# hungkq-1724/EraXviF5TTS

Measured on AMD Instinct MI355X. Metric: mel-frames/s, higher is better.
Workload: dtype bf16; 1 GPU; C2 F5TTS_Base random-init, CFM.sample euler NFE=32 CFG=2 sway=-1, 32 utterances x seq_len 1024 (N_ref=341), one GPU, hipGraph=on; global_batch=32, per_gpu_batch=32, seq_len=1024, nfe=32, parallelism=utterance-sharded dp1, residual_stream=fp16 storage, fp32 arithmetic

## Files before the change

eraxvif5tts_amd/_lib.py:

```python
from __future__ import annotations

import ctypes as C
import os

import torch

_HERE = os.path.dirname(os.path.abspath(__file__))
LIB_PATH = os.environ.get("F5HIP_LIB") or os.path.join(_HERE, "lib", "libf5hip.so")

F5_PREC_BF16, F5_PREC_FP32, F5_PREC_FP16 = 0, 1, 2
PRECISIONS = {"bf16": F5_PREC_BF16, "fp32": F5_PREC_FP32, "fp16": F5_PREC_FP16}
F5_ODE_EULER, F5_ODE_MIDPOINT, F5_ODE_RK4, F5_ODE_HEUN2, F5_ODE_HEUN3 = 0, 1, 2, 3, 4
ODE_METHODS = {"euler": F5_ODE_EULER, "midpoint": F5_ODE_MIDPOINT, "rk4": F5_ODE_RK4, "heun2": F5_ODE_HEUN2, "heun3": F5_ODE_HEUN3}
F5_ROPE_ADJACENT, F5_ROPE_HALF_SPLIT = 0, 1
F5_BACKBONE_DIT, F5_BACKBONE_UNETT, F5_BACKBONE_MMDIT = 0, 1, 2
F5_SKIP = {"concat": 0, "add": 1, "none": 2}
SITES = ("qkv", "attention", "attn_out", "ff1", "ff2", "ln1", "ln2", "conv31", "input_proj")
F5_MEL_VOCOS, F5_MEL_BIGVGAN = 0, 1
ACT = {"none": 0, "gelu_tanh": 1, "gelu_erf": 2, "mish": 3}


class F5HipError(RuntimeError):
    pass

# ... 63 lines not shown
    "f5_sample_masked": (_I, [_P, _I, _I, _P, _P, _I, _P, _P, _P, _P, _I, _F, _I, _P, _P, _P, _I, _P]),
    "f5_sample_finish": (_I, [_P, _P]),
    "f5_text_embed": (_I, [_P, _I, _I, _P, _I, _I, _P, _P]),
    "f5_dit_forward": (_I, [_P, _I, _I, _P, _P, _P, _P, _I, _P, _P, _P]),
    "f5_sample_ragged": (_I, [_P, _I, _P, _P, _P, _I, _P, _P, _P, _I, C.c_float, _I, _P, _P]),
    "f5_sample_ragged_ex": (_I, [_P, _I, _P, _P, _P, _I, _P, _P, _P, _P, _I, C.c_float, _P, _I, _P, _P]),
    "f5_mmdit_forward": (_I, [_P, _I, _I, _I, _P, _P, _P, _P, _I, _P, _P, _P]),
    "f5_cfm_noise": (_I, [_I, _I, _I, _P, _P, _P, _P, _P, _P, _P]),
    "f5_cfm_loss_workspace": (C.c_int64, [_I, _I, _I]),
    "f5_cfm_loss": (_I, [_I, _I, _I, _P, _P, _P, _P, _P, _P, _P, _P, _P]),
    "f5_distill_loss_workspace": (C.c_int64, [_I, _I, _I]),
    "f5_distill_loss": (_I, [_I, _I, _I, _P, _P, _P, _P, _P, _P, _P, _P, _P, _P]),
    "f5_plan_set_blocks": (_I, [_P, _P, _I]),
    "f5_plan_get_blocks": (_I, [_P, _P, _I]),
    "f5_align_similarity":(_I, [_I, _I, _I, _I, _I, _I, _P, _P, _P, _P, _P, _P, _P, _P]),
    "f5_align_workspace": (C.c_int64, [_I, _I, _I]),
    "f5_align_viterbi": (_I, [_I, _I, _I, _P, _P, _P, _P, _P]),
    "f5_align_window": (_I, [_I, _I, _I, _P, _P, _P, _P, _P]),
    "f5_duration_loss": (_I, [_I, _I, _P, _P, _P, _P, _P, _P, _P, _P]),
    "f5_plan_timing_begin": (_I, [_P, _I]),
    "f5_plan_timing_end": (_I, [_P, C.POINTER(C.c_float), C.POINTER(C.c_int), _P]),
    "f5_plan_timing_site": (_I, [_P, _I, C.POINTER(C.c_float), C.POINTER(C.c_int)]),
    "f5_plan_set_tap": (_I, [_P, C.c_char_p, _P]),
    "f5_plan_set_option": (_I, [_P, C.c_char_p, _I]),
    "f5_plan_set_attn_dropout": (_I, [_P, _F, C.c_uint64]),
    "f5_plan_get_option": (_I, [_P, C.c_char_p, C.POINTER(C.c_int)]),
    "f5_duration_predict": (_I, [C.POINTER(DurationWeights), _I, _I, _P, _I, _P, _P, _P, _P]),
    "f5_duration_predict_g": (_I, [C.POINTER(DurationWeights), _I, _I, _P, _I, _P, _P, _I, _P, _P, _P]),
    "f5_op_linear": (_I, [_I, _I, _I, _I, _I, _P, _P, _P, _I, _P, _P]),
    "f5_op_linear_fused": (_I, [_I, _I, _I, _I, _I, _P, _P, _P, _I, _P, _P, _P, _I, _I, _P, _P]),
    "f5_op_ln_fold": (_I, [_I, _I, _I, _I, _I, _P, _P, _P, _P, _P, _P, _P, _P, _P, _P, _I, _P, _I, _I, _P, _P, _P]),
    "f5_op_linear_fused_p": (_I, [_I, _I, _I, _I, _I, _I, _P, _P, _P, _I, _P, _P, _P, _I, _I, _P, _P]),
    "f5_op_ln_fold_p": (_I, [_I, _I, _I, _I, _I, _I, _P, _P, _P, _P, _P, _P, _P, _P, _P, _P, _I, _P, _I, _I, _P, _P, _P]),
    "f5_op_layernorm_modulate": (_I, [_I, _I, _P, _P, _P, _P, _P]),
    "f5_op_attention": (_I, [_I, _I, _I, _I, _I, _P, _P, _P, _P]),
    "f5_op_attention_dropout": (_I, [_I, _I, _I, _I, _I, _P, _P, _F, C.c_uint64, C.c_uint32, C.c_uint32, _P, _P]),
    "f5_op_attention_prescaled": (_I, [_I, _I, _I, _I, _P, _P, _P, _P]),
    "f5_op_fold_weights": (_I, [_I, _I, _I, _I, _I, _P, _P, _P, _P, _P, _P, _P, _P, _P, _P]),
    "f5_op_attention_ragged": (_I, [_I, _I, _I, _I, C.POINTER(C.c_int), C.POINTER(C.c_int), _I, _I, _I, _I, _P, _P, _P]),
    "f5_op_conv_pos_embed": (_I, [_I, _I, _I, _I, _P, _P, _P, _P, _P, _P, _P]),
    "f5_op_conv31": (_I, [_I, _I, _I, _I, _I, _P, _P, _P, _I, _P, _P]),
    "f5_op_tile_gemm": (_I, [C.POINTER(TileGemm), _P]),
    "f5_op_layernorm_res": (_I, [_I, _I, _I, _I, _I, _I, _I, _I, _P, _P, _P, _I, _P, _P, _I, _I, _I, _I, _I, _P, _P, _P, _P]),
    "f5_op_f32_to_f16": (_I, [C.c_int64, _P, _P, _P, _P]),
    "f5_op_qknorm_rope": (_I, [_I, _I, _I, _I, _I, _P, _P, _P, _P, _P, _P]),
    "f5_op_dwconv7_ln": (_I, [_I, _I, _I, _I, _P, _P, _P, _P, _P, _P, _P]),
    "f5_op_grn": (_I, [_I, _I, _I, _I, _P, _P, _P, _P, _P]),
    "f5_op_rmsnorm": (_I, [_I, _I, _I, _P, _P, _P, _P]),
    "f5_bench_gemm_site": (_I, [_I, _I, _I, _I, _I, _I, _I, _I, C.POINTER(C.c_float), _P]),
    "f5_bench_attention": (_I, [_I, _I, _I, _I, _I, C.POINTER(C.c_float), _P]),
    "f5_bench_mfma_rate": (_I, [_I, C.POINTER(C.c_float), _P]),
    "f5_tuning_set": (_I, [C.c_char_p, _I]),
    "f5_tuning_get": (_I, [C.c_char_p, C.POINTER(C.c_int)]),
    "f5_tuning_key": (C.c_char_p, [_I]),
    "f5_debug_gemm_clock": (_I, [_P]),
    "f5_debug_last_gemm": (_I, [C.POINTER(C.c_int)] * 5),
    "f5_debug_eval_modes": (_I, [_P, _I, _I, _I, C.POINTER(C.c_int32)]),
    "f5_vocoder_create": (_I, [C.POINTER(VocosConfig), C.POINTER(_P)]),
    "f5_vocoder_set_tensor": (_I, [_P, C.c_char_p, _P, C.POINTER(C.c_int64), _I]),
    "f5_vocoder_has_tensor": (_I, [_P, C.c_char_p, C.POINTER(C.c_int64)]),
    "f5_vocoder_finalize": (_I, [_P]),
    "f5_vocoder_destroy": (_I, [_P]),
    "f5_vocoder_decode": (_I, [_P, _I, _I, _P, _P, _P]),
    "f5_vocoder_istft_head": (_I, [_P, _I, _I, _P, _P, _P]),
    "f5_vocoder_decode_ragged": (_I, [_P, _I, C.POINTER(C.c_int32), C.POINTER(C.c_int32), _P, _I, _P, C.POINTER(C.c_int64), _P]),
    "f5_wave_finish": (_I, [_I, _P, C.POINTER(C.c_int32), C.POINTER(C.c_float), C.POINTER(C.c_uint8), _P, C.c_float, _I, _I, _P, _P, _P, _P, _P,
# ... 124 lines not shown
```

eraxvif5tts_amd/csrc/gemm_w4.hip:

```cpp
#include "gemm_tile.h"
#include "lnf_stats_math.h"
#include "tuning.h"
#include <string.h>

typedef _Float16 f16x4_t __attribute__((ext_vector_type(4)));

namespace {
constexpr int OPB = 32768;
constexpr int EPI_LDS_BYTES = 16384;

template <int EPI, bool LNF, int MI, typename EL = bf16_t>
__global__ __launch_bounds__(256) __attribute__((amdgpu_waves_per_eu(1, 1))) void gemm_w4_kernel(GemmParams p, int tiles_n, int nblocks) {
    static_assert(EPI == EPI_STORE_T || EPI == EPI_ROPE_T || EPI == EPI_RESID, "block linears only");
    static_assert(!LNF || EPI != EPI_RESID, "LayerNorm fold: QKV (+ RoPE) and FF1 (+ GELU)");
    static_assert(MI == 8 || MI == 4, "token tiles per wave");
    constexpr int WROWS = MI * 16, BM = 2 * WROWS;
    constexpr int OPA = BM * 128;
    constexpr int WBASE = 2 * OPA, EPI_LDS = 2 * OPA + 2 * OPB;
    constexpr int NP = MI + 8, NR = MI + 8, NMF = 16 * MI;
    constexpr int LNF_AREA = MI == 4 ? 11264 : 2048;
    constexpr int EPI_BYTES = 4 * LNF_AREA > EPI_LDS_BYTES ? 4 * LNF_AREA : EPI_LDS_BYTES;
    constexpr bool WL = MI == 8 && EPI != EPI_RESID;
    __shared__ __attribute__((aligned(1024))) char smem[EPI_LDS + EPI_BYTES];
    const int tid = threadIdx.x, lane = tid & 63;
    const int wave = __builtin_amdgcn_readfirstlane(tid >> 6);
    const int wm = wave >> 1, wn = wave & 1;
    const int fr = lane & 15, fq = lane >> 4;

    auto tile_mn = [&](int bid, int& tm0, int& tn0) {
        const int q = nblocks >> 3, r = nblocks & 7, xcd = bid & 7;
        int swz = (xcd < r ? xcd * (q + 1) : r * (q + 1) + (xcd - r) * q) + (bid >> 3);
        if (p.tile_reverse) swz = nblocks - 1 - swz;
        const int gm = p.tile_group > 0 ? p.tile_group : 1;
        const int tiles_m_all = nblocks / tiles_n;
        const int grp = swz / (gm * tiles_n);
        const int gsz = min(gm, tiles_m_all - grp * gm);
        const int rin = swz - grp * gm * tiles_n;
        const int tile_n = rin / gsz, tile_m = grp * gm + (rin - tile_n * gsz);
        tm0 = tile_m * BM;
        tn0 = tile_n * 256;
    };
    [[maybe_unused]] unsigned pfv[4] = {0u, 0u, 0u, 0u};
    if constexpr (MI == 4) {
        if (p.pf_n[0] | p.pf_n[1]) {
#pragma unroll
            for (int r = 0; r < 2; ++r) {
                const size_t line = ((size_t)blockIdx.x * 2 + r) * 256u + tid;
                if (line * 128u < p.pf_n[0]) pfv[r] = *reinterpret_cast<const unsigned*>(static_cast<const char*>(p.pf_p[0]) + line * 128u);
                if (line * 128u < p.pf_n[1]) pfv[2 + r] = *reinterpret_cast<const unsigned*>(static_cast<const char*>(p.pf_p[1]) + line * 128u);
            }
        }
    }
    const int G = gridDim.x;
    const int my_tiles = (nblocks - (int)blockIdx.x + G - 1) / G;
    const int nk = p.K / 64;

    unsigned voffA[MI], voffW[8];
#pragma unroll
    for (int jj = 0; jj < 8; ++jj) {
        const int row = (wave * 8 + jj) * 8 + (lane >> 3);
        const int logical = (lane & 7) ^ ((row >> 1) & 7);
        const int wrow = WL ? (row & ~127) + 8 * (row & 15) + ((row & 127) >> 4) : row;
        voffW[jj] = (unsigned)(wrow * p.ldw * 2 + logical * 16);
    }
#pragma unroll
    for (int jj = 0; jj < MI; ++jj) {
        const int row = (wave * MI + jj) * 8 + (lane >> 3);
        const int logical = (lane & 7) ^ ((row >> 1) & 7);
        voffA[jj] = (unsigned)(row * p.lda * 2 + logical * 16);
    }
    const char* baseA;
    const char* baseW;
    int f_tile = blockIdx.x, f_k = 0;
    auto front_tile = [&]() {
        int sm, sn;
        tile_mn(f_tile, sm, sn);
        baseA = static_cast<const char*>(p.A) + (size_t)sm * p.lda * 2;
        baseW = static_cast<const char*>(p.W) + (size_t)sn * p.ldw * 2;
    };
    front_tile();
    const unsigned lds0 = (unsigned)(size_t)smem;
    const int wdstA = (int)lds0 + wave * MI * 1024, wdstW = (int)lds0 + WBASE + wave * 8192;
    auto dma16w = [&](int ldsdst, unsigned voff, const char* base) {
        asm volatile("s_mov_b32 m0, %0\n\ts_nop 0\n\tglobal_load_lds_dwordx4 %1, %2" ::"s"(ldsdst), "v"(voff), "s"(base) : "memory");
    };
    auto dma4w = [&](int ldsdst, unsigned voff, const void* base) {
        asm volatile("s_mov_b32 m0, %0\n\ts_nop 0\n\tglobal_load_lds_dword %1, %2" ::"s"(ldsdst), "v"(voff), "s"(base) : "memory");
    };
    auto front_advance = [&]() {
        baseA += 128;
        baseW += 128;
        if (++f_k == nk) {
            f_k = 0;
            f_tile += G;
            if (f_tile < nblocks) {
// ... 1 lines not shown
            } else {
                f_tile -= G;
                baseA -= (size_t)nk * 128;
                baseW -= (size_t)nk * 128;
            }
        }
    };
    const unsigned ra0 = lds0 + (unsigned)((wm * WROWS + fr) * 128 + ((fq ^ (fr >> 1)) * 16));
    const unsigned ra1 = ra0 ^ 64u;
    const unsigned rw0 = lds0 + WBASE + (unsigned)((wn * 128 + fr) * 128 + ((fq ^ (fr >> 1)) * 16));
    const unsigned rw1 = rw0 ^ 64u;

    f32x4 acc[8][MI];
    f32x4 fw[2][8], fa[2][MI];
#define W4_DSR(dst, addr, off) asm volatile("ds_read_b128 %0, %1 offset:%2" : "=v"(dst) : "v"(addr), "n"(off))
    auto rd = [&](auto sc, auto xc, auto ec) {
        constexpr int S = decltype(sc)::value, X = decltype(xc)::value, e = decltype(ec)::value;
        (void)fw; (void)fa; (void)ra0; (void)ra1; (void)rw0; (void)rw1;
        if constexpr (e < 8) {
            if constexpr (S == 0) W4_DSR(fw[0][e], rw0, X * OPB + e * 2048); else W4_DSR(fw[1][e], rw1, X * OPB + e * 2048);
        } else {
            if constexpr (S == 0) W4_DSR(fa[0][e - 8], ra0, X * OPA + (e - 8) * 2048); else W4_DSR(fa[1][e - 8], ra1, X * OPA + (e - 8) * 2048);
        }
    };
    auto body = [&](auto xc, auto waitc) {
        constexpr int X = decltype(xc)::value;
        constexpr bool WAITV = decltype(waitc)::value;
        constexpr int R1S = 1, B1P = MI == 8 ? 20 : 13, D0 = MI == 8 ? 22 : 14, DS = MI == 8 ? 6 : 4, B2P = MI == 8 ? 86 : 42, R0 = MI == 8 ? 88 : 44,
                      R0S = MI == 8 ? 2 : 1;
        static_for<NMF>([&](auto nc) {
            (void)acc; (void)fw; (void)fa; (void)voffA; (void)voffW; (void)baseA; (void)baseW;
            constexpr int n = decltype(nc)::value;
            constexpr int s = n / (8 * MI), i = (n % (8 * MI)) / MI, j = n % MI;
            if constexpr (WL) {
                if constexpr (LNF || Elem<EL>::F16)
                    asm volatile("v_mfma_f32_16x16x32_f16 %0, %1, %2, %0" : "+a"(acc[i][j]) : "v"(fa[s][j]), "v"(fw[s][i]));
                else
                    asm volatile("v_mfma_f32_16x16x32_bf16 %0, %1, %2, %0" : "+a"(acc[i][j]) : "v"(fa[s][j]), "v"(fw[s][i]));
            } else if constexpr (LNF || Elem<EL>::F16)
                asm volatile("v_mfma_f32_16x16x32_f16 %0, %1, %2, %0" : "+a"(acc[i][j]) : "v"(fw[s][i]), "v"(fa[s][j]));
            else
                asm volatile("v_mfma_f32_16x16x32_bf16 %0, %1, %2, %0" : "+a"(acc[i][j]) : "v"(fw[s][i]), "v"(fa[s][j]));
            if constexpr (n < NR * R1S && n % R1S == 0) rd(std::integral_constant<int, 1>{}, xc, std::integral_constant<int, n / R1S>{});
            if constexpr (n == B1P) asm volatile("s_waitcnt lgkmcnt(0)\n\ts_barrier" ::: "memory");
            if constexpr (n >= D0 && n < D0 + NP * DS && (n - D0) % DS == 0) {
                constexpr int pc = (n - D0) / DS;
                if constexpr (pc < MI)
                    dma16w(X * OPA + wdstA + pc * 1024, voffA[pc], baseA);
                else
                    dma16w(X * OPB + wdstW + (pc - MI) * 1024, voffW[pc - MI], baseW);
            }
            if constexpr (n == B2P) {
                constexpr int issued = (B2P - D0) / DS + 1 > NP ? NP : (B2P - D0) / DS + 1;
                if constexpr (WAITV)
                    asm volatile("s_waitcnt vmcnt(%0)\n\ts_barrier" ::"n"(issued) : "memory");
                else
                    asm volatile("s_barrier" ::: "memory");
            }
            if constexpr (n >= R0 && n < R0 + NR * R0S && (n - R0) % R0S == 0)
                rd(std::integral_constant<int, 0>{}, std::integral_constant<int, 1 - X>{}, std::integral_constant<int, (n - R0) / R0S>{});
            if constexpr (n == NMF - 1) asm volatile("s_waitcnt lgkmcnt(0)" ::: "memory");
        });
        front_advance();
    };

    using T = std::true_type;
    using F = std::false_type;
// ... 16 lines not shown
#pragma unroll
                    for (int c = 0; c < 16; ++c)
                        dma16w(ldst + 2048 + c * 512, ro, reinterpret_cast<const char*>(p.lnf_partial + (size_t)c * p.lnf_partial_ld * 2));
                    if (p.lnf_pivot) dma16w(ldst + 2048 + 8192, ro, reinterpret_cast<const char*>(p.lnf_pivot));
                }
                return;
            }
        }
        dma16w(ldst + 1024, (unsigned)((m0 + wm * WROWS + 2 * lane) * 8), reinterpret_cast<const char*>(p.lnf_stats));
    };
    [[maybe_unused]] auto finish_stats = [&]() {
        if constexpr (MI == 4 && LNF) {
            if (p.lnf_partial) {
                float s1 = 0.f, s2 = 0.f;
#pragma unroll
                for (int c = 0; c < 16; ++c) {
                    const f32x2 v = *reinterpret_cast<const f32x2*>(lnf_lds + 2048 + c * 512 + lane * 8);
                    s1 += v[0];
                    s2 += v[1];
                }
                const float pv = p.lnf_pivot ? *reinterpret_cast<const float*>(lnf_lds + 2048 + 8192 + lane * 8) : 0.0f;
                float mean, rstd, sumsq;
                lnf_row_stats(s1, s2, pv, p.K, mean, rstd, sumsq);
                *reinterpret_cast<f32x2*>(lnf_lds + 1024 + lane * 8) = f32x2{mean, rstd};
                if (p.lnf_stats_out && n0 == 0 && wn == 0) {
                    const int m = m0 + wm * WROWS + lane;
                    const bool tok = p.lnf_rows == 0 || m + p.row0 < p.lnf_rows;
                    if (tok) *reinterpret_cast<f32x2*>(p.lnf_stats_out + (size_t)m * 2) = f32x2{mean, rstd};
                    lnf_raise_guard(p.lnf_sat, tok && !(sumsq < 65504.0f * 65504.0f), sumsq, p.lnf_sat_tag, m + p.row0);
                }
            }
        }
    };
    constexpr int NBS = WL ? 2 : 8;
    auto load_bias = [&](int tn0, f32x4 (&dst)[NBS]) {
        if constexpr (WL) {
            dst[0] = *reinterpret_cast<const f32x4*>(p.bias + tn0 + wn * 128 + 8 * fr);
            dst[1] = *reinterpret_cast<const f32x4*>(p.bias + tn0 + wn * 128 + 8 * fr + 4);
        } else {
#pragma unroll
            for (int i = 0; i < NBS; ++i) dst[i] = *reinterpret_cast<const f32x4*>(p.bias + tn0 + wn * 128 + i * 16 + 4 * fq);
        }
    };
    auto acc_from = [&](const f32x4 (&b4)[NBS]) {
        static_for<8>([&](auto ic) {
            static_for<MI>([&](auto jc) {
                constexpr int i = decltype(ic)::value;
                if constexpr (WL) {
                    const float b = b4[i >> 2][i & 3];
                    acc[i][decltype(jc)::value] = f32x4{b, b, b, b};
                } else {
                    acc[i][decltype(jc)::value] = b4[i];
                }
            });
        });
    };
#define W4_ACC(i, j)                                                                         \
    ([&]() -> f32x4 {                                                                        \
        float c0_, c1_, c2_, c3_;                                                            \
        asm volatile("v_accvgpr_read_b32 %0, %1" : "=v"(c0_) : "a"(acc[i][j][0]));           \
        asm volatile("v_accvgpr_read_b32 %0, %1" : "=v"(c1_) : "a"(acc[i][j][1]));           \
        asm volatile("v_accvgpr_read_b32 %0, %1" : "=v"(c2_) : "a"(acc[i][j][2]));           \
        asm volatile("v_accvgpr_read_b32 %0, %1" : "=v"(c3_) : "a"(acc[i][j][3]));           \
        return f32x4{c0_, c1_, c2_, c3_};                                                    \
    }())

    [[maybe_unused]] auto store_half_impl = [&](auto hc, auto actc, auto ropec) {
        constexpr int h = decltype(hc)::value, ACT = decltype(actc)::value;
        constexpr bool rope_wave = decltype(ropec)::value;
        const int nb = n0 + wn * 128 + h * 64;
        bf16_t* orow = reinterpret_cast<bf16_t*>(p.out_t) + (size_t)(m0 + wm * WROWS + fr) * p.ldo + nb + 16 * (fq & 1) + 8 * (fq >> 1);
        const size_t jstride = (size_t)16 * p.ldo;
        [[maybe_unused]] f32x4 rp[2][4];
        [[maybe_unused]] int pos0 = 0;
        auto load_rope = [&](auto jc, f32x4 (&dst)[4]) {
            constexpr int j = decltype(jc)::value;
            int pos = pos0 + 16 * j;
            pos -= pos >= p.rows_per_batch ? p.rows_per_batch : 0;
            const float* t = p.rope + (size_t)pos * 64 + 4 * fq;
#pragma unroll
            for (int i = 0; i < 4; ++i) dst[i] = *reinterpret_cast<const f32x4*>(t + 16 * i);
// ... 93 lines not shown
                *reinterpret_cast<u32x4*>(sbase + (size_t)(16 * j + r) * rstride + loff) = u32x4{q0[0], q0[1], q1[0], q1[1]};
                if constexpr (ROPE && j + 1 < MI) load_rope(16 * (j + 1) + r, rp[r]);
            });
        });
    };
    [[maybe_unused]] auto store_wave = [&](auto actc) {
        if constexpr (EPI == EPI_ROPE_T) {
            auto rotates = [&](int h) {
                const int nb = n0 + wn * 128 + h * 64;
                const int part = nb / p.rope_inner;
                return part < 2 && ((nb - part * p.rope_inner) >> 6) < p.rope_heads;
            };
            const bool r0 = rotates(0), r1 = rotates(1);
            if (r0 || r1) {
                store_wave_impl(actc, std::true_type{}, r0, r1);
                return;
            }
        }
        store_wave_impl(actc, std::false_type{}, false, false);
    };
    [[maybe_unused]] auto store_half = [&](auto hc, auto actc) {
        if constexpr (EPI == EPI_ROPE_T) {
            const int nb = n0 + wn * 128 + decltype(hc)::value * 64;
            const int part = nb / p.rope_inner;
            if (part < 2 && ((nb - part * p.rope_inner) >> 6) < p.rope_heads) {
                store_half_impl(hc, actc, std::true_type{});
                return;
            }
        }
        store_half_impl(hc, actc, std::false_type{});
    };
    [[maybe_unused]] const float* const lds_bias = reinterpret_cast<const float*>(smem + EPI_LDS);
    [[maybe_unused]] const float* const lds_gate = lds_bias + p.N;
    [[maybe_unused]] auto emit_stats = [&](int nb, int m , float pivot, const f32x4& h0, const f32x4& h1, const f32x4& h2, const f32x4& h3) {
        const f32x4 npv{-pivot, -pivot, -pivot, -pivot};
        const f32x4 d0 = h0 + npv, d1 = h1 + npv, d2 = h2 + npv, d3 = h3 + npv;
        const f32x4 a = (d0 + d1) + (d2 + d3);
        const f32x4 q = __builtin_elementwise_fma(d3, d3, __builtin_elementwise_fma(d2, d2, __builtin_elementwise_fma(d1, d1, d0 * d0)));
        const float s1 = (a[0] + a[1]) + (a[2] + a[3]), s2 = (q[0] + q[1]) + (q[2] + q[3]);
        float a0 = s1, b0 = s2;
        asm volatile("s_nop 1\n\tv_permlane16_swap_b32 %0, %1" : "+v"(a0), "+v"(b0));
        float t = a0 + b0, z = 0.0f;
        asm volatile("s_nop 1\n\tv_permlane32_swap_b32 %0, %1" : "+v"(t), "+v"(z));
        const float tot = t + z;
        if (fq < 2) {
            char* sb = reinterpret_cast<char*>(p.stats_out + ((size_t)(nb >> 6) * p.stats_ld + (m0 + wm * WROWS)) * 2);
            *reinterpret_cast<float*>(sb + (unsigned)((m * 2 + fq) * 4)) = tot;
        }
    };
    [[maybe_unused]] auto resid_tile = [&]() {
        int fr = lane & 15, fq = lane >> 4;
        asm volatile("" : "+v"(fr), "+v"(fq));
        char* const sbase = reinterpret_cast<char*>(p.out_f) + ((size_t)(m0 + wm * WROWS) * p.ldof + n0 + wn * 128) * 2;
        unsigned offj[MI];
#pragma unroll
        for (int j = 0; j < MI; ++j) offj[j] = (unsigned)(((fr + 16 * j) * p.ldof + 16 * (fq & 1) + 8 * (fq >> 1)) * 2);
        unsigned keepbits = 0xffu;
        if (p.rowmask && p.rowbits) keepbits = ((unsigned)p.rowbits[((m0 + wm * WROWS) >> 7) * 16 + fr] >> (((m0 + wm * WROWS) & 127) >> 4)) & ((1u << MI) - 1u);
        float piv[MI];
        if (p.stats_out) {
            const float* pbase = p.stats_pivot ? p.stats_pivot + (size_t)(m0 + wm * WROWS) * 2 : nullptr;
#pragma unroll
            for (int j = 0; j < MI; ++j) piv[j] = pbase ? *reinterpret_cast<const float*>(reinterpret_cast<const char*>(pbase) + (unsigned)((fr + 16 * j) * 8)) : 0.0f;
        }
        u32x4 xs[2][MI][2];
        auto load_step = [&](auto sc) __attribute__((always_inline)) {
            constexpr int h = decltype(sc)::value / MI, j = decltype(sc)::value % MI;
// ... 22 lines not shown
                constexpr int h = decltype(sc)::value / MI, j = decltype(sc)::value % MI;
                const int nb = n0 + wn * 128 + h * 64;
                if constexpr (j == 0) {
#pragma unroll
                    for (int ii = 0; ii < 4; ++ii) g4[ii] = *reinterpret_cast<const f32x4*>(lds_gate + nb + ii * 16 + 4 * fq);
                }
                f32x4 x0, x1, x2, x3;
                {
                    const u32x4 q = xs[h][j][0];
                    const u32x2 s0 = __builtin_amdgcn_permlane16_swap(q[0], q[2], false, false);
                    const u32x2 s1 = __builtin_amdgcn_permlane16_swap(q[1], q[3], false, false);
                    x0 = widen_h(s0[0], s1[0]);
                    x1 = widen_h(s0[1], s1[1]);
                }
                {
                    const u32x4 q = xs[h][j][1];
                    const u32x2 s0 = __builtin_amdgcn_permlane16_swap(q[0], q[2], false, false);
                    const u32x2 s1 = __builtin_amdgcn_permlane16_swap(q[1], q[3], false, false);
                    x2 = widen_h(s0[0], s1[0]);
                    x3 = widen_h(s0[1], s1[1]);
                }
                const f32x4 a0 = W4_ACC(h * 4 + 0, j), a1 = W4_ACC(h * 4 + 1, j), a2 = W4_ACC(h * 4 + 2, j), a3 = W4_ACC(h * 4 + 3, j);
                f32x4 v0 = epi_axpy4(a0, g4[0], x0), v1 = epi_axpy4(a1, g4[1], x1), v2 = epi_axpy4(a2, g4[2], x2), v3 = epi_axpy4(a3, g4[3], x3);
                if constexpr (!ALL) {
                    const bool keep = (keepbits >> j) & 1u;
                    v0 = keep ? v0 : x0;
                    v1 = keep ? v1 : x1;
                    v2 = keep ? v2 : x2;
                    v3 = keep ? v3 : x3;
                }
                const f16x4_t h0 = to_h16(v0), h1 = to_h16(v1), h2 = to_h16(v2), h3 = to_h16(v3);
                *reinterpret_cast<u32x4*>(sbase + offj[j] + h * 128) = pair_swap(__builtin_bit_cast(bf16x4, h0), __builtin_bit_cast(bf16x4, h1));
                *reinterpret_cast<u32x4*>(sbase + offj[j] + h * 128 + 64) = pair_swap(__builtin_bit_cast(bf16x4, h2), __builtin_bit_cast(bf16x4, h3));
                if (p.stats_out) emit_stats(nb, fr + 16 * j, piv[j], h_f32(h0), h_f32(h1), h_f32(h2), h_f32(h3));
                if constexpr (decltype(sc)::value + AHEAD < 2 * MI) load_step(std::integral_constant<int, decltype(sc)::value + AHEAD>{});
                __builtin_amdgcn_sched_barrier(0);
            });
        };
        if (all_kept)
            steps(std::true_type{});
        else
            steps(std::false_type{});
    };

    if constexpr (EPI == EPI_RESID) {
        float* lb = reinterpret_cast<float*>(smem + EPI_LDS);
        for (int i = tid; i < p.N; i += 256) {
            lb[i] = p.bias[i];
            lb[p.N + i] = p.gate ? p.gate[i] : 1.0f;
        }
    }
    auto issue_all = [&](int X) {
#pragma unroll
        for (int pc = 0; pc < MI; ++pc) dma16w(X * OPA + wdstA + pc * 1024, voffA[pc], baseA);
#pragma unroll
        for (int pc = 0; pc < 8; ++pc) dma16w(X * OPB + wdstW + pc * 1024, voffW[pc], baseW);
    };
    if constexpr (LNF) stage_lnf();
    issue_all(0);
    front_advance();
    issue_all(1);
    front_advance();
    f32x4 bstart[NBS];
    if constexpr (LNF) {
#pragma unroll
        for (int i = 0; i < NBS; ++i) bstart[i] = f32x4{0.f, 0.f, 0.f, 0.f};
    } else {
        load_bias(n0, bstart);
        if constexpr (WL) {
#pragma unroll
            for (int i = 0; i < NBS; ++i) asm volatile("" ::"v"(bstart[i]));
        }
    }
    acc_from(bstart);
    if constexpr (EPI == EPI_RESID) asm volatile("s_waitcnt lgkmcnt(0)" ::: "memory");
    asm volatile("s_waitcnt vmcnt(%0)\n\ts_barrier" ::"n"(NP) : "memory");
    static_for<NR>([&](auto ec) { rd(std::integral_constant<int, 0>{}, std::integral_constant<int, 0>{}, ec); });
    asm volatile("s_waitcnt lgkmcnt(0)" ::: "memory");

    for (int t = 0; t < my_tiles; ++t) {
        const bool last = t + 1 == my_tiles;
        if (t == 0)
            body(X0{}, T{});
        else
            body(X0{}, F{});
        body(X1{}, T{});
        for (int kt = 2; kt < nk; kt += 2) {
            body(X0{}, T{});
            body(X1{}, T{});
        }
        int nm0 = m0, nn0 = n0;
        if (!last) tile_mn(blockIdx.x + (t + 1) * G, nm0, nn0);
        if constexpr (EPI == EPI_RESID) {
            asm volatile("s_waitcnt vmcnt(0)" ::: "memory");
            __builtin_amdgcn_sched_barrier(0);
            resid_tile();
            __builtin_amdgcn_sched_barrier(0);
            f32x4 bn[8];
#pragma unroll
            for (int i = 0; i < 8; ++i) bn[i] = *reinterpret_cast<const f32x4*>(lds_bias + nn0 + wn * 128 + i * 16 + 4 * fq);
            acc_from(bn);
        } else {
            f32x4 bn[NBS];
            if constexpr (LNF) {
#pragma unroll
                for (int i = 0; i < NBS; ++i) bn[i] = f32x4{0.f, 0.f, 0.f, 0.f};
            } else {
                load_bias(nn0, bn);
#pragma unroll
                for (int i = 0; i < NBS; ++i) asm volatile("" ::"v"(bn[i]));
            }
            asm volatile("s_waitcnt vmcnt(0)" ::: "memory");
            __builtin_amdgcn_sched_barrier(0);
            finish_stats();
            if constexpr (WL) {
                if (p.act == ACT_GELU_TANH)
                    store_wave(std::integral_constant<int, ACT_GELU_TANH>{});
                else
                    store_wave(std::integral_constant<int, ACT_NONE>{});
            } else if (p.act == ACT_GELU_TANH) {
                store_half(X0{}, std::integral_constant<int, ACT_GELU_TANH>{});
                store_half(X1{}, std::integral_constant<int, ACT_GELU_TANH>{});
            } else {
                store_half(X0{}, std::integral_constant<int, ACT_NONE>{});
                store_half(X1{}, std::integral_constant<int, ACT_NONE>{});
            }
            __builtin_amdgcn_sched_barrier(0);
            acc_from(bn);
        }
        m0 = nm0;
        n0 = nn0;
        if (!last) {
            static_for<NR>([&](auto ec) { rd(std::integral_constant<int, 0>{}, std::integral_constant<int, 0>{}, ec); });
// ... 94 lines not shown
```

eraxvif5tts_amd/csrc/ops.hip:

```cpp
#include <cstring>

#include "gemm.h"
#include "kernels.h"
#include "model_internal.h"
#include "runtime.h"
#include "tuning.h"

static int sync_and_release(DevArena& a, hipStream_t st, int rc) {
    hipError_t e = hipStreamSynchronize(st);
    a.release();
    if (rc != 0) return rc;
    if (e != hipSuccess) return f5_fail(F5_EHIP, "stream synchronize failed: %s", hipGetErrorString(e));
    return 0;
}

extern "C" int f5_op_linear(int precision, int kernel, int M, int N, int K, const float* A, const float* W, const float* bias, int act,
                            float* out, f5_stream_t stream) {
    F5_TRY(f5_check_device());
    if (M <= 0 || N <= 0 || K <= 0 || !A || !W || !out) return f5_fail(F5_EINVAL, "bad argument");
    hipStream_t st = (hipStream_t)stream;
    const int Kp = (int)round_up(K, 64), Mp = (int)round_up(M, 256), Np = (int)round_up(N, 256);
    const size_t es = f5_elem_size(precision);
    DevArena a;
    void *At = nullptr, *Wt = nullptr;
// ... 90 lines not shown
        if ((rc = a.alloc_t(&c2, (size_t)N))) break;
        if ((rc = launch_convert_pad(precision, A, Kb, M, Kb, Kb, At, Kb, st))) break;
        if ((rc = launch_convert_pad(precision, Wo, Kb, D, Kb, Kb, Wot, Kb, st))) break;
        if ((rc = launch_f32_to_f16(x, xs, (size_t)M * D, st))) break;
        if (pivot) F5_HIP(hipMemcpyAsync(st2, pivot, (size_t)M * 2 * sizeof(float), hipMemcpyDeviceToDevice, st));
        F5_HIP(hipMemcpyAsync(mod, shift, (size_t)D * sizeof(float), hipMemcpyDeviceToDevice, st));
        F5_HIP(hipMemcpyAsync(mod + D, scale, (size_t)D * sizeof(float), hipMemcpyDeviceToDevice, st));
        GemmParams g;
        memset(&g, 0, sizeof(g));
        g.A = At; g.lda = Kb; g.W = Wot; g.ldw = Kb; g.M = M; g.N = D; g.K = Kb; g.bias = bo; g.rows_per_batch = seq > 0 ? seq : M;
        g.out_f = reinterpret_cast<float*>(xs); g.ldof = D; g.add2_f16 = 1; g.gate = gate;
        g.stats_out = partial; g.stats_ld = (int)Mp; g.stats_pivot = pivot ? st2 : nullptr;
        if ((rc = launch_gemm(g, precision, GEMM_DENSE, EPI_RESID, 1, st))) break;
        if ((rc = launch_stats_finalize(partial, (int)Mp, D / 64, M, D, pivot ? st2 : nullptr, st2, nullptr, 0, st))) break;
        if ((rc = launch_fold_weights(W, bias, mod, 6 * D, 1, 1, N, N, D, Wt, c1, c2, st))) break;
        memset(&g, 0, sizeof(g));
        g.A = xs; g.lda = D; g.W = Wt; g.ldw = D; g.M = M; g.N = N; g.K = D; g.act = act; g.out_t = Ot; g.ldo = N; g.rows_per_batch = seq > 0 ? seq : M;
        g.lnf_stats = st2; g.lnf_c1 = c1; g.lnf_c2 = c2;
        if (epi == EPI_ROPE_T) { g.rope = rope; g.rope_inner = N / 3; g.rope_heads = rope_heads; }
        if ((rc = launch_gemm(g, precision, GEMM_DENSE, epi, 1, st))) break;
        if ((rc = launch_f16_to_f32(xs, x, (size_t)M * D, st))) break;
        F5_HIP(hipMemcpyAsync(stats, st2, (size_t)M * 2 * sizeof(float), hipMemcpyDeviceToDevice, st));
        rc = launch_convert_back(precision, Ot, N, M, N, out, N, st);
    } while (0);
    return sync_and_release(a, st, rc);
}

extern "C" int f5_op_ln_fold(int epi, int M, int D, int N, int Kb, float* x, const float* A, const float* Wo, const float* bo, const float* gate,
                             const float* pivot, const float* W, const float* bias, const float* scale, const float* shift, int act,
                             const float* rope, int rope_heads, int seq, float* stats, float* out, f5_stream_t stream) {
    return f5_op_ln_fold_p(F5_PREC_BF16, epi, M, D, N, Kb, x, A, Wo, bo, gate, pivot, W, bias, scale, shift, act, rope, rope_heads, seq, stats, out, stream);
}

extern "C" int f5_op_layernorm_modulate(int rows, int dim, const float* x, const float* scale, const float* shift, float* out,
                                        f5_stream_t stream) {
    F5_TRY(f5_check_device());
    if (!x || !scale || !shift || !out) return f5_fail(F5_EINVAL, "null argument");
    return launch_layernorm(F5_PREC_FP32, x, dim, rows, dim, scale, shift, 0, rows, 1, out, dim, (hipStream_t)stream);
}

extern "C" int f5_op_attention(int precision, int kernel, int B, int N, int H, const float* qkv, const uint8_t* mask, float* out,
                               f5_stream_t stream) {
    F5_TRY(f5_check_device());
    if (B <= 0 || N <= 0 || H <= 0 || !qkv || !out) return f5_fail(F5_EINVAL, "bad argument");
    hipStream_t st = (hipStream_t)stream;
    const int inner = H * 64, rows = B * N;
    const size_t es = f5_elem_size(precision);
    DevArena a;
    void *q = nullptr, *o = nullptr;
    int rc = 0;
    do {
        if ((rc = a.alloc(&q, (size_t)rows * 3 * inner * es))) break;
        if ((rc = a.alloc(&o, (size_t)rows * inner * es))) break;
        if ((rc = launch_convert_pad(precision, qkv, 3 * inner, rows, 3 * inner, 3 * inner, q, 3 * inner, st))) break;
        if ((rc = launch_attention(precision, kernel, B, N, H, q, 3 * inner, mask, o, inner, st))) break;
        rc = launch_convert_back(precision, o, inner, rows, inner, out, inner, st);
    } while (0);
    return sync_and_release(a, st, rc);
}

extern "C" int f5_op_attention_dropout(int precision, int kernel, int B, int N, int H, const float* qkv, const uint8_t* mask, float prob, uint64_t seed,
                                       uint32_t stream_word, uint32_t batch0, float* out, f5_stream_t stream) {
    if (!(prob >= 0.f && prob < 1.f)) return f5_fail(F5_EINVAL, "f5_op_attention_dropout: prob must lie in [0, 1)");
    if (prob == 0.f) return f5_op_attention(precision, kernel, B, N, H, qkv, mask, out, stream);
    F5_TRY(f5_check_device());
    if (B <= 0 || N <= 0 || H <= 0 || !qkv || !out) return f5_fail(F5_EINVAL, "bad argument");
// ... 617 lines not shown
```

include/f5hip.h:

```cpp
#ifndef F5HIP_H
#define F5HIP_H

#include <stdint.h>

#ifdef __cplusplus
extern "C" {
#endif

#define F5_API __attribute__((visibility("default")))

#define F5HIP_VERSION 400

#define F5_OK 0
#define F5_EINVAL -1
#define F5_ENODEVICE -2
#define F5_EHIP -3
#define F5_ESTATE -4
#define F5_ENOTSUP -5
#define F5_ENOMEM -6

#define F5_PREC_BF16 0
#define F5_PREC_FP32 1
#define F5_PREC_FP16 2

// ... 112 lines not shown
#define F5_SITE_COUNT 9
F5_API int f5_plan_timing_site(f5_plan_t p, int site, float* avg_ms, int* launches);
F5_API int f5_plan_set_option(f5_plan_t p, const char* key, int value);
F5_API int f5_plan_get_option(f5_plan_t p, const char* key, int* value);
F5_API int f5_plan_set_attn_dropout(f5_plan_t p, float prob, uint64_t seed);
F5_API int f5_plan_set_blocks(f5_plan_t p, const int32_t* blocks_host, int count);
F5_API int f5_plan_get_blocks(f5_plan_t p, int32_t* blocks_host, int cap);

typedef struct f5_duration_weights {
    const float *text_embed, *conv1_w, *conv1_b, *norm1_w, *norm1_b, *conv2_w, *conv2_b, *norm2_w, *norm2_b, *proj_w, *proj_b;
    int32_t vocab_rows, in_channels, filter_channels, kernel_size;
    const float *cond_w, *cond_b;
    int32_t gin_channels;
} f5_duration_weights;
F5_API int f5_duration_predict(const f5_duration_weights* w, int batch, int nt, const int32_t* tokens, int add_one, const int32_t* mask,
                        float* scratch, float* out, f5_stream_t stream);
F5_API int f5_duration_predict_g(const f5_duration_weights* w, int batch, int nt, const int32_t* tokens, int add_one, const int32_t* mask,
                          const float* g, int g_nt, float* scratch, float* out, f5_stream_t stream);

F5_API int f5_op_linear(int precision, int kernel, int M, int N, int K, const float* A, const float* W, const float* bias, int act,
                 float* out, f5_stream_t stream);
F5_API int f5_op_linear_fused(int kernel, int epi, int M, int N, int K, const float* A, const float* W, const float* bias, int act,
                       const float* gate, const uint8_t* rowmask, const float* rope, int rope_heads, int seq, float* out,
                       f5_stream_t stream);
F5_API int f5_op_linear_fused_p(int precision, int kernel, int epi, int M, int N, int K, const float* A, const float* W, const float* bias, int act,
                         const float* gate, const uint8_t* rowmask, const float* rope, int rope_heads, int seq, float* out,
                         f5_stream_t stream);
F5_API int f5_op_ln_fold(int epi, int M, int D, int N, int Kb, float* x, const float* A, const float* Wo, const float* bo, const float* gate,
                         const float* pivot, const float* W, const float* bias, const float* scale, const float* shift, int act, const float* rope,
                         int rope_heads, int seq, float* stats, float* out, f5_stream_t stream);
F5_API int f5_op_ln_fold_p(int precision, int epi, int M, int D, int N, int Kb, float* x, const float* A, const float* Wo, const float* bo,
                           const float* gate, const float* pivot, const float* W, const float* bias, const float* scale, const float* shift, int act,
                           const float* rope, int rope_heads, int seq, float* stats, float* out, f5_stream_t stream);
F5_API int f5_op_layernorm_modulate(int rows, int dim, const float* x, const float* scale, const float* shift, float* out,
                             f5_stream_t stream);
F5_API int f5_op_attention(int precision, int kernel, int B, int N, int H, const float* qkv, const uint8_t* mask, float* out,
                    f5_stream_t stream);
F5_API int f5_op_attention_dropout(int precision, int kernel, int B, int N, int H, const float* qkv, const uint8_t* mask, float prob,
                                   uint64_t seed, uint32_t stream_word, uint32_t batch0, float* out, f5_stream_t stream);
F5_API int f5_op_attention_prescaled(int kernel, int B, int N, int H, const float* qkv, const uint8_t* mask, float* out, f5_stream_t stream);
F5_API int f5_op_fold_weights(int R, int qkv_rows, int q_rows, int D, int qscaled, const float* W, const float* bias, const float* scale_msa,
                              const float* shift_msa, const float* scale_mlp, const float* shift_mlp, float* Wt, float* c1, float* c2,
                              f5_stream_t stream);
F5_API int f5_op_attention_ragged(int precision, int attn_kernel, int nbr, int cnt, const int* off, const int* n, int H, int rows,
                                  int ldq_extra, int ldo_extra, const float* qkv, float* out, f5_stream_t stream);
F5_API int f5_op_conv_pos_embed(int precision, int B, int N, int dim, const float* x, const float* w0, const float* b0,
                         const float* w1, const float* b1, float* out, f5_stream_t stream);
F5_API int f5_op_conv31(int precision, int kernel, int B, int N, int dim, const float* x, const float* w, const float* b, int act, float* out,
                        f5_stream_t stream);
typedef struct f5_tile_gemm {
    const float *A, *W, *bias, *gate, *rope, *addend;
    const uint8_t* rowmask;
    float *out_t, *out_f;
    int32_t precision, mode, epi, M, N, K, a_row_mod, act, gate_bstride, rows_per_batch, rope_heads, ldadd, add2_f16, ldo, ldof, out_rows;
} f5_tile_gemm;
F5_API int f5_op_tile_gemm(const f5_tile_gemm* g, f5_stream_t stream);

F5_API int f5_op_layernorm_res(int precision, int xin_f16, int xout_f16, int rows, int dim, int ldx, int ldy, int ldo, const float* x,
                               const float* y, const float* y2, int ymode, const float* mul, const float* add, int mod_bstride,
                               int rows_per_batch, int add_one, int inplace, int sat_tag, float* out, float* xback, uint32_t* guard,
                               f5_stream_t stream);
F5_API int f5_op_f32_to_f16(int64_t n, const float* src, float* dst, uint32_t* guard, f5_stream_t stream);
F5_API int f5_op_qknorm_rope(int precision, int rows, int heads, int rope_heads, int rows_per_batch, const float* qkv, const float* wq,
                             const float* wk, const float* rope, float* out, f5_stream_t stream);
F5_API int f5_op_dwconv7_ln(int precision, int B, int N, int C, const float* x, const float* wt, const float* cbias, const float* ln_w,
                            const float* ln_b, float* out, f5_stream_t stream);
// ... 164 lines not shown
```

Measured before the change: 36270 mel-frames/s.

## Use swizzled weight layout and LDS-patch stats epilogue for MI=8 residual GEMM

Extends the interleaved weight-row layout and the two-bias-vector accumulator initialisation, previously used only by the MI=8 non-residual GEMMs, to the MI=8 residual (attn_out/ff2) GEMM. It adds a new residual epilogue that writes fp16 results straight to global memory while staging them in a per-wave LDS patch, then reads them back transposed to compute LayerNorm statistics. It also adds a standalone test entry point for the residual-plus-stats path. The aim is better MFMA operand layout and cheaper stats emission, at the cost of 16 KB of extra LDS and more complex epilogue scheduling.

```diff
diff --git a/eraxvif5tts_amd/_lib.py b/eraxvif5tts_amd/_lib.py
--- a/eraxvif5tts_amd/_lib.py
+++ b/eraxvif5tts_amd/_lib.py
@@ -119,6 +119,7 @@
     "f5_op_ln_fold": (_I, [_I, _I, _I, _I, _I, _P, _P, _P, _P, _P, _P, _P, _P, _P, _P, _I, _P, _I, _I, _P, _P, _P]),
     "f5_op_linear_fused_p": (_I, [_I, _I, _I, _I, _I, _I, _P, _P, _P, _I, _P, _P, _P, _I, _I, _P, _P]),
     "f5_op_ln_fold_p": (_I, [_I, _I, _I, _I, _I, _I, _P, _P, _P, _P, _P, _P, _P, _P, _P, _P, _I, _P, _I, _I, _P, _P, _P]),
+    "f5_op_resid_stats_p": (_I, [_I, _I, _I, _I, _P, _P, _P, _P, _P, _P, _P, _P, _P, _P, _P]),
     "f5_op_layernorm_modulate": (_I, [_I, _I, _P, _P, _P, _P, _P]),
     "f5_op_attention": (_I, [_I, _I, _I, _I, _I, _P, _P, _P, _P]),
     "f5_op_attention_dropout": (_I, [_I, _I, _I, _I, _I, _P, _P, _F, C.c_uint64, C.c_uint32, C.c_uint32, _P, _P]),
diff --git a/eraxvif5tts_amd/csrc/gemm_w4.hip b/eraxvif5tts_amd/csrc/gemm_w4.hip
--- a/eraxvif5tts_amd/csrc/gemm_w4.hip
+++ b/eraxvif5tts_amd/csrc/gemm_w4.hip
@@ -21,7 +21,10 @@
     constexpr int LNF_AREA = MI == 4 ? 11264 : 2048;
     constexpr int EPI_BYTES = 4 * LNF_AREA > EPI_LDS_BYTES ? 4 * LNF_AREA : EPI_LDS_BYTES;
     constexpr bool WL = MI == 8 && EPI != EPI_RESID;
-    __shared__ __attribute__((aligned(1024))) char smem[EPI_LDS + EPI_BYTES];
+    constexpr bool RL = MI == 8 && EPI == EPI_RESID;
+    constexpr bool SWP = WL || RL;
+    constexpr int PATCH = EPI_LDS + EPI_BYTES, PATCH_BYTES = RL ? 4 * 4096 : 0;
+    __shared__ __attribute__((aligned(4096))) char smem[EPI_LDS + EPI_BYTES + PATCH_BYTES];
     const int tid = threadIdx.x, lane = tid & 63;
     const int wave = __builtin_amdgcn_readfirstlane(tid >> 6);
     const int wm = wave >> 1, wn = wave & 1;
@@ -60,7 +63,7 @@
     for (int jj = 0; jj < 8; ++jj) {
         const int row = (wave * 8 + jj) * 8 + (lane >> 3);
         const int logical = (lane & 7) ^ ((row >> 1) & 7);
-        const int wrow = WL ? (row & ~127) + 8 * (row & 15) + ((row & 127) >> 4) : row;
+        const int wrow = SWP ? (row & ~127) + 8 * (row & 15) + ((row & 127) >> 4) : row;
         voffW[jj] = (unsigned)(wrow * p.ldw * 2 + logical * 16);
     }
 #pragma unroll
@@ -128,7 +131,7 @@
             (void)acc; (void)fw; (void)fa; (void)voffA; (void)voffW; (void)baseA; (void)baseW;
             constexpr int n = decltype(nc)::value;
             constexpr int s = n / (8 * MI), i = (n % (8 * MI)) / MI, j = n % MI;
-            if constexpr (WL) {
+            if constexpr (SWP) {
                 if constexpr (LNF || Elem<EL>::F16)
                     asm volatile("v_mfma_f32_16x16x32_f16 %0, %1, %2, %0" : "+a"(acc[i][j]) : "v"(fa[s][j]), "v"(fw[s][i]));
                 else
@@ -211,9 +214,9 @@
             }
         }
     };
-    constexpr int NBS = WL ? 2 : 8;
+    constexpr int NBS = SWP ? 2 : 8;
     auto load_bias = [&](int tn0, f32x4 (&dst)[NBS]) {
-        if constexpr (WL) {
+        if constexpr (SWP) {
             dst[0] = *reinterpret_cast<const f32x4*>(p.bias + tn0 + wn * 128 + 8 * fr);
             dst[1] = *reinterpret_cast<const f32x4*>(p.bias + tn0 + wn * 128 + 8 * fr + 4);
         } else {
@@ -225,7 +228,7 @@
         static_for<8>([&](auto ic) {
             static_for<MI>([&](auto jc) {
                 constexpr int i = decltype(ic)::value;
-                if constexpr (WL) {
+                if constexpr (SWP) {
                     const float b = b4[i >> 2][i & 3];
                     acc[i][decltype(jc)::value] = f32x4{b, b, b, b};
                 } else {
@@ -385,7 +388,7 @@
     };
     [[maybe_unused]] const float* const lds_bias = reinterpret_cast<const float*>(smem + EPI_LDS);
     [[maybe_unused]] const float* const lds_gate = lds_bias + p.N;
-    [[maybe_unused]] auto emit_stats = [&](int nb, int m , float pivot, const f32x4& h0, const f32x4& h1, const f32x4& h2, const f32x4& h3) {
+    [[maybe_unused]] auto emit_stats = [&](int fq , int nb, int m , float pivot, const f32x4& h0, const f32x4& h1, const f32x4& h2, const f32x4& h3) {
         const f32x4 npv{-pivot, -pivot, -pivot, -pivot};
         const f32x4 d0 = h0 + npv, d1 = h1 + npv, d2 = h2 + npv, d3 = h3 + npv;
         const f32x4 a = (d0 + d1) + (d2 + d3);
@@ -474,8 +477,110 @@
                 const f16x4_t h0 = to_h16(v0), h1 = to_h16(v1), h2 = to_h16(v2), h3 = to_h16(v3);
                 *reinterpret_cast<u32x4*>(sbase + offj[j] + h * 128) = pair_swap(__builtin_bit_cast(bf16x4, h0), __builtin_bit_cast(bf16x4, h1));
                 *reinterpret_cast<u32x4*>(sbase + offj[j] + h * 128 + 64) = pair_swap(__builtin_bit_cast(bf16x4, h2), __builtin_bit_cast(bf16x4, h3));
-                if (p.stats_out) emit_stats(nb, fr + 16 * j, piv[j], h_f32(h0), h_f32(h1), h_f32(h2), h_f32(h3));
+                if (p.stats_out) emit_stats(fq, nb, fr + 16 * j, piv[j], h_f32(h0), h_f32(h1), h_f32(h2), h_f32(h3));
                 if constexpr (decltype(sc)::value + AHEAD < 2 * MI) load_step(std::integral_constant<int, decltype(sc)::value + AHEAD>{});
+                __builtin_amdgcn_sched_barrier(0);
+            });
+        };
+        if (all_kept)
+            steps(std::true_type{});
+        else
+            steps(std::false_type{});
+    };
+
+    [[maybe_unused]] auto resid_tile_wl = [&]() {
+        int lid = (int)__builtin_amdgcn_mbcnt_hi(~0u, __builtin_amdgcn_mbcnt_lo(~0u, 0u));
+        asm volatile("" : "+v"(lid));
+        const int fc = lid & 15, fq = lid >> 4;
+        typedef __attribute__((address_space(1))) char gchar;
+        typedef __attribute__((address_space(1))) u32x4 gu32x4;
+        gchar* sst = (gchar*)(reinterpret_cast<char*>(p.out_f) + ((size_t)(m0 + wm * WROWS) * p.ldof + n0 + wn * 128) * 2);
+        const gchar* sld = sst;
+        const size_t jstride = (size_t)p.ldof * 32;
+        unsigned offr[4];
+#pragma unroll
+        for (int r = 0; r < 4; ++r) offr[r] = (unsigned)(((4 * fq + r) * p.ldof + 8 * fc) * 2);
+        unsigned kb4 = 0xffffffffu;
+        if (p.rowmask && p.rowbits) kb4 = *reinterpret_cast<const unsigned*>(p.rowbits + ((m0 + wm * WROWS) >> 7) * 16 + 4 * fq);
+        const int fq_st = p.stats_out ? fq : 4;
+        float piv[MI];
+#pragma unroll
+        for (int j = 0; j < MI; ++j) piv[j] = 0.0f;
+        if (p.stats_out && p.stats_pivot) {
+            const char* pbase = reinterpret_cast<const char*>(p.stats_pivot + (size_t)(m0 + wm * WROWS) * 2);
+#pragma unroll
+            for (int j = 0; j < MI; ++j) piv[j] = *reinterpret_cast<const float*>(pbase + (unsigned)((fc + 16 * j) * 8));
+        }
+        char* const patch = smem + PATCH + wave * 4096;
+        const unsigned wof = (unsigned)(4 * fq * 256 + ((fc ^ (4 * fq)) * 16));
+        const unsigned rof = (unsigned)(fc * 256 + ((fc >> 1) & 7) * 32 + (((fq >> 1) ^ (fc & 1)) * 16) + (fq & 1) * 8);
+        constexpr int AHEAD = 6;
+        u32x4 xs[4 * MI];
+        auto load_step = [&](auto sc) __attribute__((always_inline)) {
+            constexpr int r = decltype(sc)::value % 4;
+            xs[decltype(sc)::value] = *(const gu32x4*)(sld + offr[r]);
+            if constexpr (r == 3) {
+                sld += jstride;
+                asm volatile("" : "+s"(sld));
+            }
+        };
+        const f32x4 g0 = *reinterpret_cast<const f32x4*>(lds_gate + n0 + wn * 128 + 8 * fc), g1 = *reinterpret_cast<const f32x4*>(lds_gate + n0 + wn * 128 + 8 * fc + 4);
+        static_for<AHEAD>([&](auto sc) { load_step(sc); });
+        __builtin_amdgcn_sched_barrier(0);
+        asm volatile("" ::"v"(g0), "v"(g1));
+        const bool all_kept = __builtin_amdgcn_ballot_w64(kb4 != 0xffffffffu) == 0ull;
+        auto widen_h = [](unsigned lo, unsigned hi) __attribute__((always_inline)) {
+            const f16x4_t hv = __builtin_bit_cast(f16x4_t, u32x2{lo, hi});
+            return f32x4{(float)hv[0], (float)hv[1], (float)hv[2], (float)hv[3]};
+        };
+        auto to_h16 = [](const f32x4& v) __attribute__((always_inline)) {
+            f16x4_t hv;
+#pragma unroll
+            for (int e = 0; e < 4; ++e) hv[e] = (_Float16)__builtin_amdgcn_fmed3f(v[e], -65504.0f, 65504.0f);
+            return hv;
+        };
+        u32x2 rb[8];
+        auto read_back = [&]() __attribute__((always_inline)) {
+#pragma unroll
+            for (int hi = 0; hi < 8; ++hi) rb[hi] = *reinterpret_cast<const u32x2*>(patch + (rof ^ (unsigned)(hi * 32)));
+        };
+        auto stats_of = [&](int j) __attribute__((always_inline)) {
+#pragma unroll
+            for (int h = 0; h < 2; ++h)
+                emit_stats(fq_st, n0 + wn * 128 + h * 64, fc + 16 * j, piv[j], widen_h(rb[h * 4][0], rb[h * 4][1]), widen_h(rb[h * 4 + 1][0], rb[h * 4 + 1][1]),
+                           widen_h(rb[h * 4 + 2][0], rb[h * 4 + 2][1]), widen_h(rb[h * 4 + 3][0], rb[h * 4 + 3][1]));
+        };
+        auto steps = [&](auto keptc) __attribute__((always_inline)) {
+            constexpr bool ALL = decltype(keptc)::value;
+            static_for<MI>([&](auto jc) __attribute__((always_inline)) {
+                constexpr int j = decltype(jc)::value;
+                __builtin_amdgcn_sched_barrier(0);
+                asm volatile("" : "+v"(offr[0]), "+v"(offr[1]), "+v"(offr[2]), "+v"(offr[3]));
+                f32x4 a[8];
+                static_for<8>([&](auto ic) { a[decltype(ic)::value] = W4_ACC(decltype(ic)::value, j); });
+                static_for<4>([&](auto rc) __attribute__((always_inline)) {
+                    constexpr int r = decltype(rc)::value, s = 4 * j + r;
+                    const u32x4 x = xs[s];
+                    const f32x4 x0 = widen_h(x[0], x[1]), x1 = widen_h(x[2], x[3]);
+                    f32x4 v0 = epi_axpy4(f32x4{a[0][r], a[1][r], a[2][r], a[3][r]}, g0, x0), v1 = epi_axpy4(f32x4{a[4][r], a[5][r], a[6][r], a[7][r]}, g1, x1);
+                    if constexpr (!ALL) {
+                        const bool keep = (kb4 >> (8 * r + j)) & 1u;
+                        v0 = keep ? v0 : x0;
+                        v1 = keep ? v1 : x1;
+                    }
+                    const u32x2 q0 = __builtin_bit_cast(u32x2, to_h16(v0)), q1 = __builtin_bit_cast(u32x2, to_h16(v1));
+                    const u32x4 q{q0[0], q0[1], q1[0], q1[1]};
+                    *(gu32x4*)(sst + offr[r]) = q;
+                    *reinterpret_cast<u32x4*>(patch + (wof ^ (unsigned)(16 * r)) + 256 * r) = q;
+                    if constexpr (s + AHEAD < 4 * MI) load_step(std::integral_constant<int, s + AHEAD>{});
+                });
+                sst += jstride;
+                asm volatile("" : "+s"(sst));
+                __builtin_amdgcn_sched_barrier(0);
+                if constexpr (j > 0) stats_of(j - 1);
+                __builtin_amdgcn_sched_barrier(0);
+                read_back();
+                if constexpr (j == MI - 1) stats_of(j);
                 __builtin_amdgcn_sched_barrier(0);
             });
         };
@@ -509,7 +614,7 @@
         for (int i = 0; i < NBS; ++i) bstart[i] = f32x4{0.f, 0.f, 0.f, 0.f};
     } else {
         load_bias(n0, bstart);
-        if constexpr (WL) {
+        if constexpr (SWP) {
 #pragma unroll
             for (int i = 0; i < NBS; ++i) asm volatile("" ::"v"(bstart[i]));
         }
@@ -536,11 +641,22 @@
         if constexpr (EPI == EPI_RESID) {
             asm volatile("s_waitcnt vmcnt(0)" ::: "memory");
             __builtin_amdgcn_sched_barrier(0);
-            resid_tile();
+            if constexpr (RL)
+                resid_tile_wl();
+            else
+                resid_tile();
             __builtin_amdgcn_sched_barrier(0);
-            f32x4 bn[8];
-#pragma unroll
-            for (int i = 0; i < 8; ++i) bn[i] = *reinterpret_cast<const f32x4*>(lds_bias + nn0 + wn * 128 + i * 16 + 4 * fq);
+            f32x4 bn[NBS];
+            if constexpr (RL) {
+                int fc = lane & 15;
+                asm volatile("" : "+v"(fc));
+                bn[0] = *reinterpret_cast<const f32x4*>(lds_bias + nn0 + wn * 128 + 8 * fc);
+                bn[1] = *reinterpret_cast<const f32x4*>(lds_bias + nn0 + wn * 128 + 8 * fc + 4);
+                asm volatile("" ::"v"(bn[0]), "v"(bn[1]));
+            } else {
+#pragma unroll
+                for (int i = 0; i < NBS; ++i) bn[i] = *reinterpret_cast<const f32x4*>(lds_bias + nn0 + wn * 128 + i * 16 + 4 * fq);
+            }
             acc_from(bn);
         } else {
             f32x4 bn[NBS];
diff --git a/eraxvif5tts_amd/csrc/ops.hip b/eraxvif5tts_amd/csrc/ops.hip
--- a/eraxvif5tts_amd/csrc/ops.hip
+++ b/eraxvif5tts_amd/csrc/ops.hip
@@ -146,6 +146,53 @@
     return f5_op_ln_fold_p(F5_PREC_BF16, epi, M, D, N, Kb, x, A, Wo, bo, gate, pivot, W, bias, scale, shift, act, rope, rope_heads, seq, stats, out, stream);
 }
 
+extern "C" int f5_op_resid_stats_p(int precision, int M, int N, int K, float* x, const float* A, const float* W, const float* bias, const float* gate,
+                                   const uint8_t* rowmask, const float* pivot, float* planes, float* stats, unsigned* guard, f5_stream_t stream) {
+    F5_TRY(f5_check_device());
+    if (precision != F5_PREC_BF16 && precision != F5_PREC_FP16) return f5_fail(F5_EINVAL, "f5_op_resid_stats_p: a 16-bit precision mode (bf16 0, fp16 2), got %d", precision);
+    if (M <= 0 || N <= 0 || K <= 0 || !x || !A || !W || !bias || !planes || !stats) return f5_fail(F5_EINVAL, "bad argument");
+    if (N % 128 != 0 || K % 32 != 0) return f5_fail(F5_EINVAL, "f5_op_resid_stats_p: N % 128, K % 32");
+    hipStream_t st = (hipStream_t)stream;
+    const size_t Mp = round_up(M, 256) + 256;
+    DevArena a;
+    void *At = nullptr, *Wt = nullptr, *xs = nullptr;
+    float *partial = nullptr, *st2 = nullptr;
+    unsigned* sat = nullptr;
+    uint8_t* bits = nullptr;
+    int rc = 0;
+    do {
+        if ((rc = a.alloc(&At, Mp * K * 2))) break;
+        if ((rc = a.alloc(&Wt, (size_t)round_up(N, 256) * K * 2))) break;
+        if ((rc = a.alloc(&xs, Mp * N * 2))) break;
+        if ((rc = a.alloc_t(&partial, (size_t)(N / 64) * Mp * 2))) break;
+        if ((rc = a.alloc_t(&st2, Mp * 2))) break;
+        if ((rc = a.alloc_t(&sat, (size_t)8))) break;
+        if ((rc = a.alloc_t(&bits, (size_t)(Mp / 128 + 1) * 16))) break;
+        if ((rc = launch_convert_pad(precision, A, K, M, K, K, At, K, st))) break;
+        if ((rc = launch_convert_pad(precision, W, K, N, K, K, Wt, K, st))) break;
+        if ((rc = launch_f32_to_f16(x, xs, (size_t)M * N, st))) break;
+        F5_HIP(hipMemsetAsync(partial, 0, (size_t)(N / 64) * Mp * 2 * sizeof(float), st));
+        F5_HIP(hipMemsetAsync(sat, 0, 8 * sizeof(unsigned), st));
+        if (pivot) F5_HIP(hipMemcpyAsync(st2, pivot, (size_t)M * 2 * sizeof(float), hipMemcpyDeviceToDevice, st));
+        GemmParams g;
+        memset(&g, 0, sizeof(g));
+        g.A = At; g.lda = K; g.W = Wt; g.ldw = K; g.M = M; g.N = N; g.K = K; g.bias = bias; g.rows_per_batch = M;
+        g.out_f = reinterpret_cast<float*>(xs); g.ldof = N; g.add2_f16 = 1; g.gate = gate;
+        g.stats_out = partial; g.stats_ld = (int)Mp; g.stats_pivot = pivot ? st2 : nullptr;
+        if (rowmask) {
+            if ((rc = launch_rowbits(rowmask, M, bits, st))) break;
+            g.rowmask = rowmask; g.rowbits = bits;
+        }
+        if ((rc = launch_gemm(g, precision, GEMM_DENSE, EPI_RESID, 1, st))) break;
+        if ((rc = launch_stats_finalize(partial, (int)Mp, N / 64, M, N, pivot ? st2 : nullptr, st2, sat, 0, st))) break;
+        if ((rc = launch_f16_to_f32(xs, x, (size_t)M * N, st))) break;
+        F5_HIP(hipMemcpy2DAsync(planes, (size_t)M * 2 * sizeof(float), partial, Mp * 2 * sizeof(float), (size_t)M * 2 * sizeof(float), N / 64, hipMemcpyDeviceToDevice, st));
+        F5_HIP(hipMemcpyAsync(stats, st2, (size_t)M * 2 * sizeof(float), hipMemcpyDeviceToDevice, st));
+        if (guard) F5_HIP(hipMemcpyAsync(guard, sat, 6 * sizeof(unsigned), hipMemcpyDeviceToDevice, st));
+    } while (0);
+    return sync_and_release(a, st, rc);
+}
+
 extern "C" int f5_op_layernorm_modulate(int rows, int dim, const float* x, const float* scale, const float* shift, float* out,
                                         f5_stream_t stream) {
     F5_TRY(f5_check_device());
diff --git a/include/f5hip.h b/include/f5hip.h
--- a/include/f5hip.h
+++ b/include/f5hip.h
@@ -168,6 +168,8 @@
 F5_API int f5_op_ln_fold_p(int precision, int epi, int M, int D, int N, int Kb, float* x, const float* A, const float* Wo, const float* bo,
                            const float* gate, const float* pivot, const float* W, const float* bias, const float* scale, const float* shift, int act,
                            const float* rope, int rope_heads, int seq, float* stats, float* out, f5_stream_t stream);
+F5_API int f5_op_resid_stats_p(int precision, int M, int N, int K, float* x, const float* A, const float* W, const float* bias, const float* gate,
+                               const uint8_t* rowmask, const float* pivot, float* planes, float* stats, unsigned* guard, f5_stream_t stream);
 F5_API int f5_op_layernorm_modulate(int rows, int dim, const float* x, const float* scale, const float* shift, float* out,
                              f5_stream_t stream);
 F5_API int f5_op_attention(int precision, int kernel, int B, int N, int H, const float* qkv, const uint8_t* mask, float* out,
```

After: 36760 mel-frames/s, median of 6. 1.4% higher.
